# al-mcintyre/mCaller

Hardware: NVIDIA B200
Metric: per-read site calls/sec (higher is better)
Workload: dtype f64

## Files before the change

include/mcaller_b200.h:

```cpp
#ifndef MCALLER_B200_H
#define MCALLER_B200_H

#include <stdint.h>

#ifdef __cplusplus
extern "C" {
#endif

#define MC_ABI_VERSION 3

#define MC_TILE_BYTES 3840
#define MC_TEXT_PAD 4096
#define MC_MAXK 8

enum {
    MC_OK = 0,
    MC_EINVAL = -1,
    MC_ECUDA = -2,
    MC_ECAPACITY = -3
};

typedef struct mc_refindex {
    int32_t n_contigs;
    int32_t k;
// ... 96 lines not shown
    const int32_t *d_feature;
    const double *d_threshold;
    const double *d_leaf_p1;
} mc_model;

typedef struct mc_qual_entry {
    uint64_t hash;
    uint32_t check;
    uint32_t len;
    double qual;
} mc_qual_entry;


int mc_version(void);
int mc_sizeof(int what);
const char *mc_last_error(void);

int mc_read_u64(const uint64_t *d_src, int64_t n, uint64_t *h_dst, void *stream);

int mc_scan(const uint8_t *d_text, int64_t nbytes, const mc_refindex *ref, int dense,
            mc_record *d_rec, int64_t rec_cap, uint32_t *d_tile_tab , uint32_t *d_run_tab ,
            uint64_t *d_counters, void *stream);

int mc_scan_run_len(int64_t nbytes);

int mc_scan_set_run_len(int run_len);

int64_t mc_num_tiles(int64_t nbytes);

int64_t mc_workspace_bytes(int64_t n);

int mc_order_records(const uint8_t *d_text, int64_t nbytes, const mc_refindex *ref, const uint32_t *d_tile_tab, int64_t n_tiles,
                     uint32_t *d_run_tab, int run_len, const mc_record *d_rec_in, int64_t rec_in_cap, const uint64_t *d_scan_counters,
                     mc_record *d_rec_out, int64_t rec_out_cap, uint64_t *d_n_out, uint32_t *d_seg_flags ,
                     uint32_t *d_run_first , void *d_ws, void *stream);

int mc_segment_reads(const uint8_t *d_text, mc_record *d_rec, const uint64_t *d_n_records, int64_t rec_cap,
                     uint32_t *d_seg_flags , const uint32_t *d_run_first, int64_t n_runs,
                     uint32_t *d_seg_start, uint64_t *d_nseg, void *d_ws, void *stream);

int mc_segment_quality(const uint8_t *d_text, const mc_record *d_rec, const uint32_t *d_seg_start, const uint64_t *d_nseg,
                       int64_t seg_cap, const mc_qual_entry *d_table, int64_t table_size, double *d_seg_qual, uint64_t *d_err,
                       void *stream);

int mc_build_windows(const mc_record *d_rec, const uint64_t *d_n_records, int64_t rec_cap, const uint32_t *d_seg_start,
                     const uint64_t *d_nseg, int64_t seg_cap, const double *d_seg_qual, const mc_refindex *ref, int skip_thresh,
                     double qual_thresh, int two_models, mc_call *d_calls, int64_t call_cap, uint32_t *d_seg_count,
                     uint64_t *d_ncalls, void *d_ws, double *d_spill, int64_t spill_cap, void *stream);

typedef struct mc_carry {
    mc_call row;
    uint32_t valid;
    int32_t first_kept_contig;
    uint64_t chunks;
    uint64_t pad[6];
} mc_carry;
int mc_carry_reset(mc_carry *d_carry, void *stream);
int mc_carry_rows(mc_call *d_rows, const uint64_t *d_ncalls, const mc_record *d_rec, const uint64_t *d_n_records,
                  const uint32_t *d_seg_start, const uint64_t *d_nseg, const double *d_seg_qual, double qual_thresh,
                  mc_carry *d_carry, uint64_t *d_nrows_out, const uint64_t *d_abort, void *stream);
int mc_chunk_guard(const uint64_t *d_counters, int64_t rec_cap, const uint64_t *d_n_records, int64_t rec_out_cap,
                   const uint64_t *d_nseg, int64_t seg_cap, const uint64_t *d_ncalls, int64_t call_cap, uint64_t *d_abort,
                   uint64_t *d_sticky , void *stream);
int mc_carry_close(mc_carry *d_carry, int closing_contig, const int64_t *d_next_contigs, int from, int count, mc_call *d_row_out,
                   uint32_t *d_depth, uint32_t *d_meth, uint64_t *d_first, int64_t n_sites, uint64_t *d_row_base, void *stream);

int64_t mc_classify_workspace_bytes(int64_t row_cap);
int mc_classify(mc_call *d_calls, const uint64_t *d_nrows, int64_t row_cap, const mc_model *models, void *d_ws, void *stream);

int mc_hist_accumulate(const mc_call *d_calls, const uint64_t *d_nrows, int64_t row_cap, uint32_t *d_depth, uint32_t *d_meth,
                       uint64_t *d_first, int64_t n_sites, uint64_t *d_row_base, mc_call *d_odd, int64_t odd_cap, uint64_t *d_n_odd,
                       const uint64_t *d_abort , void *stream);
// ... 91 lines not shown
```

mcaller_b200/_lib.py:

```python
import ctypes as C
import os

import numpy as np

HERE = os.path.dirname(os.path.abspath(__file__))
LIB_PATH = os.environ.get("MCALLER_B200_LIB") or os.path.join(HERE, "libmcaller_b200.so")

MC_TILE_BYTES = 3840
MC_TEXT_PAD = 4096
MC_MAXK = 8
MC_C_COUNT = 16
COUNTER_NAMES = ["lines", "kept", "records", "short", "unknown_contig", "nnn", "badpos", "longline", "overflow", "run_cursor", "quiet_chunks"]

MC_ABI_VERSION = 3
MC_CALL, MC_TOO_MANY_SKIPS, MC_MULTI_M, MC_NONE = 0, 1, 2, 3
MC_CE_CONTEXT, MC_CE_MODELKEY, MC_CE_BADNUM, MC_CE_COLUMN, MC_CE_SPACING = 1, 2, 4, 8, 16
MC_MLP, MC_LR, MC_GNB, MC_RF = 0, 1, 2, 3
PENDING = 0xFFFFFFFF


class RefIndex(C.Structure):
    _fields_ = [("n_contigs", C.c_int32), ("k", C.c_int32), ("d_names", C.c_void_p), ("d_name_off", C.c_void_p),
                ("d_base", C.c_void_p), ("d_len", C.c_void_p), ("d_site_fwd", C.c_void_p), ("d_site_rev", C.c_void_p),
                ("d_cand", C.c_void_p), ("d_rank_fwd", C.c_void_p), ("d_rank_rev", C.c_void_p), ("d_bases", C.c_void_p),
# ... 36 lines not shown
                ("lr", C.c_double), ("tol", C.c_double), ("best_loss", C.c_double), ("n_iter", C.c_int32), ("no_improve", C.c_int32),
                ("stopped", C.c_int32), ("pad", C.c_int32)]


MC_TRAIN_HIDDEN, MC_TRAIN_BATCH = 100, 200

CARRY_BYTES = 192

QUAL_DTYPE = np.dtype([("hash", "<u8"), ("check", "<u4"), ("len", "<u4"), ("qual", "<f8")])
assert QUAL_DTYPE.itemsize == 24
DIFFS_ROW_DTYPE = np.dtype([("line_off", "<u8"), ("slot", "<u4"), ("values_off", "<u4"), ("values_len", "<u4"), ("prob_off", "<u4"),
                            ("prob_len", "<u4"), ("pad", "<u4")])
assert DIFFS_ROW_DTYPE.itemsize == 32


class McallerCudaError(RuntimeError):
    pass


_lib = None

_PROTOS = {
    "mc_version": (C.c_int, []),
    "mc_sizeof": (C.c_int, [C.c_int]),
    "mc_last_error": (C.c_char_p, []),
    "mc_read_u64": (C.c_int, [C.c_void_p, C.c_int64, C.c_void_p, C.c_void_p]),
    "mc_scan": (C.c_int, [C.c_void_p, C.c_int64, C.POINTER(RefIndex), C.c_int, C.c_void_p, C.c_int64, C.c_void_p, C.c_void_p, C.c_void_p,
                          C.c_void_p]),
    "mc_scan_run_len": (C.c_int, [C.c_int64]),
    "mc_scan_set_run_len": (C.c_int, [C.c_int]),
    "mc_num_tiles": (C.c_int64, [C.c_int64]),
    "mc_workspace_bytes": (C.c_int64, [C.c_int64]),
    "mc_order_records": (C.c_int, [C.c_void_p, C.c_int64, C.POINTER(RefIndex), C.c_void_p, C.c_int64, C.c_void_p, C.c_int, C.c_void_p,
                                   C.c_int64, C.c_void_p, C.c_void_p, C.c_int64, C.c_void_p, C.c_void_p, C.c_void_p, C.c_void_p, C.c_void_p]),
    "mc_segment_reads": (C.c_int, [C.c_void_p, C.c_void_p, C.c_void_p, C.c_int64, C.c_void_p, C.c_void_p, C.c_int64, C.c_void_p, C.c_void_p,
                                   C.c_void_p, C.c_void_p]),
    "mc_segment_quality": (C.c_int, [C.c_void_p, C.c_void_p, C.c_void_p, C.c_void_p, C.c_int64, C.c_void_p, C.c_int64, C.c_void_p,
                                     C.c_void_p, C.c_void_p]),
    "mc_build_windows": (C.c_int, [C.c_void_p, C.c_void_p, C.c_int64, C.c_void_p, C.c_void_p, C.c_int64, C.c_void_p, C.POINTER(RefIndex),
                                   C.c_int, C.c_double, C.c_int, C.c_void_p, C.c_int64, C.c_void_p, C.c_void_p, C.c_void_p, C.c_void_p,
                                   C.c_int64, C.c_void_p]),
    "mc_carry_reset": (C.c_int, [C.c_void_p, C.c_void_p]),
    "mc_carry_rows": (C.c_int, [C.c_void_p, C.c_void_p, C.c_void_p, C.c_void_p, C.c_void_p, C.c_void_p, C.c_void_p, C.c_double, C.c_void_p,
                                C.c_void_p, C.c_void_p, C.c_void_p]),
    "mc_chunk_guard": (C.c_int, [C.c_void_p, C.c_int64, C.c_void_p, C.c_int64, C.c_void_p, C.c_int64, C.c_void_p, C.c_int64, C.c_void_p,
                                 C.c_void_p, C.c_void_p]),
    "mc_carry_close": (C.c_int, [C.c_void_p, C.c_int, C.c_void_p, C.c_int, C.c_int, C.c_void_p, C.c_void_p, C.c_void_p, C.c_void_p,
                                 C.c_int64, C.c_void_p, C.c_void_p]),
    "mc_classify_workspace_bytes": (C.c_int64, [C.c_int64]),
    "mc_classify": (C.c_int, [C.c_void_p, C.c_void_p, C.c_int64, C.POINTER(Model), C.c_void_p, C.c_void_p]),
    "mc_hist_accumulate": (C.c_int, [C.c_void_p, C.c_void_p, C.c_int64, C.c_void_p, C.c_void_p, C.c_void_p, C.c_int64, C.c_void_p,
                                     C.c_void_p, C.c_int64, C.c_void_p, C.c_void_p, C.c_void_p]),
    "mc_count_calls": (C.c_int, [C.c_void_p, C.c_void_p, C.c_int64, C.c_void_p, C.c_void_p]),
    "mc_bed_select": (C.c_int, [C.c_void_p, C.c_void_p, C.c_int64, C.c_int64, C.c_double, C.c_int, C.c_void_p, C.c_void_p, C.c_void_p]),
    "mc_format_rows": (C.c_int64, [C.c_void_p, C.c_int64, C.c_void_p, C.c_void_p, C.c_int32, C.c_void_p, C.c_void_p, C.c_void_p, C.c_void_p,
                                   C.c_int32, C.c_int32, C.c_char_p, C.c_char_p, C.c_int32, C.c_int32, C.c_void_p, C.c_int64]),
    "mc_fastq_tiles": (C.c_int64, [C.c_int64]),
    "mc_fastq_index": (C.c_int, [C.c_void_p, C.c_int64, C.c_void_p, C.c_void_p, C.c_void_p, C.c_int64, C.c_void_p, C.c_void_p, C.c_void_p]),
    "mc_fastq_quality": (C.c_int, [C.c_void_p, C.c_int64, C.c_void_p, C.c_int64, C.c_void_p, C.c_int64, C.c_void_p, C.c_void_p, C.c_void_p,
                                   C.c_void_p]),
    "mc_synth_genome": (C.c_int, [C.POINTER(SynthSpec), C.c_void_p, C.c_int64, C.c_void_p]),
    "mc_synth_sizes": (C.c_int, [C.POINTER(SynthSpec), C.c_int64, C.c_int64, C.c_int64, C.c_void_p, C.c_void_p]),
    "mc_synth_write": (C.c_int, [C.POINTER(SynthSpec), C.c_int64, C.c_int64, C.c_int64, C.c_void_p, C.c_void_p, C.c_void_p]),
    "mc_diffs_aggregate_ex": (C.c_int, [C.c_void_p, C.c_int64, C.c_int64, C.c_void_p, C.c_int64, C.c_void_p, C.c_int64, C.c_void_p, C.c_void_p]),
    "mc_diffs_rehash": (C.c_int, [C.c_void_p, C.c_int64, C.c_void_p, C.c_int64, C.c_void_p, C.c_void_p]),
    "mc_diffs_rows": (C.c_int, [C.c_void_p, C.c_int64, C.c_void_p, C.c_int64, C.c_void_p, C.c_int64, C.c_void_p, C.c_int64, C.c_void_p,
                                C.c_void_p]),
    "mc_mlp_train_init": (C.c_int, [C.c_void_p, C.c_int32, C.c_void_p]),
    "mc_mlp_train_epochs": (C.c_int, [C.c_void_p, C.c_int32, C.c_void_p, C.c_int32, C.c_void_p]),
# ... 31 lines not shown
```

mcaller_b200/csrc/records.cu:

```cuda
#include "parse.cuh"

namespace {

constexpr int SCAN_THREADS = 256;
constexpr int SCAN_IPT = 8;
constexpr int SCAN_BLOCK = SCAN_THREADS * SCAN_IPT;

__global__ void __launch_bounds__(SCAN_THREADS) k_scan_reduce(const uint32_t *__restrict__ in, int64_t n_cap,
                                                            const unsigned long long *__restrict__ d_n,
                                                            unsigned long long *__restrict__ block_sums) {
    __shared__ int s_warp[SCAN_THREADS / 32 + 1];
    const int64_t n = d_n ? mc_dev_count(d_n, n_cap) : n_cap;
    const int64_t base = (int64_t)blockIdx.x * SCAN_BLOCK;
    unsigned long long acc = 0ull;
#pragma unroll
    for (int j = 0; j < SCAN_IPT; ++j) {
        const int64_t i = base + (int64_t)j * SCAN_THREADS + threadIdx.x;
        if (i < n) acc += in[i];
    }
    for (int d = 16; d > 0; d >>= 1) acc += __shfl_down_sync(0xffffffffu, acc, d);
    __shared__ unsigned long long s_sum[SCAN_THREADS / 32];
    if ((threadIdx.x & 31) == 0) s_sum[threadIdx.x >> 5] = acc;
    __syncthreads();
    if (threadIdx.x == 0) {
// ... 59 lines not shown
    int total;
    int off = mc_block_exscan<SCAN_THREADS>(sum, s_warp, total);
    uint32_t run = (uint32_t)block_sums[blockIdx.x] + (uint32_t)off;
#pragma unroll
    for (int j = 0; j < SCAN_IPT; ++j) {
        const int64_t i = base + j;
        if (i < n) out[i] = run;
        run += v[j];
    }
}

}

int64_t mc_exscan_ws_bytes(int64_t n) { return ((n + SCAN_BLOCK - 1) / SCAN_BLOCK + 1) * 8 + 256; }

int mc_exscan_u32(const uint32_t *d_in, uint32_t *d_out, int64_t n_cap, const uint64_t *d_n, uint64_t *d_total, void *d_ws,
                  cudaStream_t st) {
    if (n_cap <= 0) {
        if (d_total) MC_CUDA_CHECK(cudaMemsetAsync(d_total, 0, 8, st));
        return MC_OK;
    }
    const int64_t nb = (n_cap + SCAN_BLOCK - 1) / SCAN_BLOCK;
    unsigned long long *sums = reinterpret_cast<unsigned long long *>(d_ws);
    const unsigned long long *dn = reinterpret_cast<const unsigned long long *>(d_n);
    k_scan_reduce<<<(unsigned)nb, SCAN_THREADS, 0, st>>>(d_in, n_cap, dn, sums);
    MC_LAUNCH_CHECK();
    k_scan_sums<<<1, 1024, 0, st>>>(sums, nb, reinterpret_cast<unsigned long long *>(d_total));
    MC_LAUNCH_CHECK();
    k_scan_down<<<(unsigned)nb, SCAN_THREADS, 0, st>>>(d_in, n_cap, dn, sums, d_out);
    MC_LAUNCH_CHECK();
    return MC_OK;
}

extern "C" int64_t mc_windows_workspace_bytes(int64_t rec_cap);
extern "C" int64_t mc_workspace_bytes(int64_t n) {
    if (n < 1) n = 1;
    const int64_t a = ((n * 4 + 255) / 256) * 256;
    const int64_t mine = 2 * a + mc_exscan_ws_bytes(n) + 512;
    const int64_t win = mc_windows_workspace_bytes(n);
    return mine > win ? mine : win;
}
static inline uint32_t *ws_a(void *ws) { return reinterpret_cast<uint32_t *>(ws); }
static inline uint32_t *ws_b(void *ws, int64_t n) { return reinterpret_cast<uint32_t *>(reinterpret_cast<uint8_t *>(ws) + ((n * 4 + 255) / 256) * 256); }
static inline void *ws_s(void *ws, int64_t n) { return reinterpret_cast<uint8_t *>(ws) + 2 * (((n * 4 + 255) / 256) * 256); }

namespace {

__global__ void __launch_bounds__(256) k_run_resolve(uint32_t *__restrict__ run_tab, int64_t n_runs, uint32_t *__restrict__ cnt_clean,
                                                    const unsigned long long *__restrict__ scan_counters, unsigned long long rec_in_cap) {
    const int64_t r = (int64_t)blockIdx.x * blockDim.x + threadIdx.x;
    if (r >= n_runs) return;
    if (scan_counters && (scan_counters[MC_C_OVERFLOW] != 0ull || scan_counters[MC_C_RECORDS] > rec_in_cap)) {
        cnt_clean[r] = 0u;
        return;
    }
    uint32_t count = run_tab[2 * r];
    const uint32_t v = run_tab[2 * r + 1];
    if (v & 1u) {
        int64_t p = r - 1;
        uint32_t st = 0u;
        while (p >= 0 && (st = (run_tab[2 * p + 1] >> 1) & 3u) == 0u) --p;
        if (p >= 0 && st == 1u && count > 0u) {
            run_tab[2 * r + 1] = v | 0x80000000u;
            --count;
        }
    }
    cnt_clean[r] = count;
}

__global__ void __launch_bounds__(256, 4) k_gather_finish(const uint8_t *__restrict__ text, int64_t limit, mc_refindex R,
                                                      const uint32_t *__restrict__ tile_tab, const uint32_t *__restrict__ run_tab,
                                                      const uint32_t *__restrict__ run_dst, int64_t n_tiles, int64_t n_runs, int run_len,
                                                      const mc_record *__restrict__ in, unsigned long long in_cap, mc_record *__restrict__ out,
                                                      unsigned long long out_cap, uint32_t *__restrict__ seg_flags,
                                                      uint32_t *__restrict__ run_first) {
    const int lane = threadIdx.x & 31;
    const int64_t warp0 = ((int64_t)blockIdx.x * blockDim.x + threadIdx.x) >> 5, n_warps = ((int64_t)gridDim.x * blockDim.x) >> 5;
    for (int64_t run = warp0; run < n_runs; run += n_warps) {
    const uint32_t rv = __ldg(run_tab + 2 * run + 1);
    const bool empty_run = __ldg(run_dst + run) == __ldg(run_dst + run + 1);
    if (run_first && lane == 0) run_first[run] = empty_run ? 0xFFFFFFFFu : __ldg(run_dst + run);
    if (__ldg(run_tab + 2 * run) == 0u) continue;
    const bool drop = (rv >> 31) != 0u;
    unsigned long long d_run = __ldg(run_dst + run);
    const int64_t c0 = run * run_len, c1 = min(c0 + (int64_t)run_len, n_tiles);
    long long carry_line = -1;
    uint32_t carry_span = 0u;
    for (int64_t cb = c0; cb < c1; cb += 32) {
        const int64_t c = cb + lane;
        unsigned long long src = 0ull;
        uint32_t cnt = 0u;
        if (c < c1) {
            const uint2 e = __ldg(reinterpret_cast<const uint2 *>(tile_tab) + c);
            src = e.x;
            cnt = e.y & 0xFFFFu;
            if (drop && ((e.y >> 16) & 1u) && cnt > 0u) { src += 1ull; --cnt; }
        }
        uint32_t incl = cnt;
#pragma unroll
        for (int d = 1; d < 32; d <<= 1) {
            const uint32_t t = __shfl_up_sync(0xffffffffu, incl, d);
            if (lane >= d) incl += t;
        }
        const uint32_t excl = incl - cnt, tot = __shfl_sync(0xffffffffu, incl, 31);
        for (uint32_t k0 = 0; k0 < tot; k0 += 32) {
            const uint32_t idx = k0 + lane;
            const bool act = idx < tot;
            int lo = 0, hi = 31;
#pragma unroll
            for (int st = 0; st < 5; ++st) {
                const int mid = (lo + hi + 1) >> 1;
                const uint32_t e_mid = __shfl_sync(0xffffffffu, excl, mid);
                if (e_mid <= idx) lo = mid; else hi = mid - 1;
            }
            const unsigned long long s_own = __shfl_sync(0xffffffffu, src, lo);
            const uint32_t e_own = __shfl_sync(0xffffffffu, excl, lo);
            const unsigned long long slot = s_own + (idx - e_own), dst = d_run + idx;
            const bool ok = act && slot < in_cap && dst < out_cap;
            alignas(16) mc_record r;
            long long line = -1;
            uint32_t span = 0u;
            if (ok) {
                const uint4 *sp = reinterpret_cast<const uint4 *>(in + slot);
                uint4 *dr = reinterpret_cast<uint4 *>(&r);
                dr[0] = __ldg(sp);
                dr[1] = __ldg(sp + 1);
                if (r.flags & MC_RF_RAW) mc_finish_record_win(text, limit, r);
                if (r.flags & MC_RF_CAND) {
                    const int cid = r.contig;
                    if (r.pos < __ldg(R.d_len + cid)) {
                        const int64_t g = __ldg(R.d_base + cid) + r.pos;
                        r.kbits_fwd = (uint8_t)mc_kmer_bits(R.d_site_fwd, g, R.k);
                        r.kbits_rev = (uint8_t)mc_kmer_bits(R.d_site_rev, g, R.k);
                    }
                }
                line = mc_rec_line(r);
                span = (uint32_t)r.name_off | ((uint32_t)r.name_len << 16);
            }
            long long pl = __shfl_up_sync(0xffffffffu, line, 1);
            uint32_t ps = __shfl_up_sync(0xffffffffu, span, 1);
            if (lane == 0) { pl = carry_line; ps = carry_span; }
            if (ok) {
                uint32_t sf = 1u;
                if (pl >= 0) {
                    uint32_t fl = r.flags | MC_RF_SEGKNOWN;
                    sf = 0u;
                    if ((ps >> 16) != r.name_len || bytes_differ(text + pl + (ps & 0xFFFFu), text + line + r.name_off, r.name_len)) {
                        fl |= MC_RF_NEWREAD;
                        sf = 1u;
                    }
                    r.flags = (uint8_t)fl;
                }
                if (seg_flags) seg_flags[dst] = sf;
                uint4 *dp = reinterpret_cast<uint4 *>(out + dst);
                const uint4 *sr = reinterpret_cast<const uint4 *>(&r);
                dp[0] = sr[0];
                dp[1] = sr[1];
            }
            const int last = (int)min(tot - k0, 32u) - 1;
            carry_line = __shfl_sync(0xffffffffu, line, last);
            carry_span = __shfl_sync(0xffffffffu, span, last);
        }
        d_run += tot;
    }
    }
}

__global__ void __launch_bounds__(256) k_seg_flags(const uint8_t *__restrict__ text, mc_record *__restrict__ rec, int64_t n_cap,
                                                  const unsigned long long *__restrict__ d_n, uint32_t *__restrict__ flags,
                                                  const uint32_t *__restrict__ known) {
    const int64_t n = mc_dev_count(d_n, n_cap);
    const int64_t i = (int64_t)blockIdx.x * blockDim.x + threadIdx.x;
    if (i >= n) return;
    if (known) {
        const uint32_t kf = known[i];
        if (kf < 2u) { flags[i] = kf; return; }
    }
    uint32_t f = 1u;
    const mc_record b = rec[i];
    if (b.flags & MC_RF_SEGKNOWN) {
        f = (b.flags & MC_RF_NEWREAD) ? 1u : 0u;
    } else {
        if (i > 0) {
            const mc_record a = rec[i - 1];
            if (a.name_len == b.name_len)
                f = bytes_differ(text + mc_rec_line(a) + a.name_off, text + mc_rec_line(b) + b.name_off, a.name_len) ? 1u : 0u;
        }
        rec[i].flags = (uint8_t)(b.flags | MC_RF_SEGKNOWN | (f ? MC_RF_NEWREAD : 0u));
    }
    flags[i] = f;
}

__global__ void __launch_bounds__(256) k_seg_fix(const uint8_t *__restrict__ text, mc_record *__restrict__ rec, const unsigned long long *__restrict__ d_n,
                                                int64_t n_cap, const uint32_t *__restrict__ run_first, int64_t n_runs, uint32_t *__restrict__ flags) {
    const int64_t run = (int64_t)blockIdx.x * blockDim.x + threadIdx.x;
    if (run >= n_runs) return;
    const uint32_t i = run_first[run];
    if (i == 0xFFFFFFFFu || (int64_t)i >= mc_dev_count(d_n, n_cap)) return;
    uint32_t f = 1u;
    const mc_record b = rec[i];
    if (i > 0u) {
        const mc_record a = rec[i - 1];
        if (a.name_len == b.name_len)
            f = bytes_differ(text + mc_rec_line(a) + a.name_off, text + mc_rec_line(b) + b.name_off, a.name_len) ? 1u : 0u;
    }
    rec[i].flags = (uint8_t)(b.flags | MC_RF_SEGKNOWN | (f ? MC_RF_NEWREAD : 0u));
    flags[i] = f;
}

__global__ void __launch_bounds__(256) k_seg_starts(const uint32_t *__restrict__ flags, const uint32_t *__restrict__ excl, int64_t n_cap,
                                                   const unsigned long long *__restrict__ d_n, uint32_t *__restrict__ seg_start,
                                                   const unsigned long long *__restrict__ d_nseg) {
    const int64_t n = mc_dev_count(d_n, n_cap);
    const int64_t i = (int64_t)blockIdx.x * blockDim.x + threadIdx.x;
    if (i < n && flags[i]) seg_start[excl[i]] = (uint32_t)i;
    if (i == 0) seg_start[*d_nseg] = (uint32_t)n;
}

__global__ void __launch_bounds__(256) k_seg_quality(const uint8_t *__restrict__ text, const mc_record *__restrict__ rec,
                                                    const uint32_t *__restrict__ seg_start, int64_t seg_cap,
                                                    const unsigned long long *__restrict__ d_nseg,
                                                    const mc_qual_entry *__restrict__ table, unsigned long long mask,
                                                    double *__restrict__ seg_qual, unsigned long long *__restrict__ d_err) {
    const int64_t n_seg = mc_dev_count(d_nseg, seg_cap);
    const int64_t s = (int64_t)blockIdx.x * blockDim.x + threadIdx.x;
    if (s >= n_seg) return;
    const mc_record r = rec[seg_start[s]];
    const mc_read_key key = mc_read_key_of(text + mc_rec_line(r) + r.name_off, r.name_len);
    double q = __longlong_as_double(0x7ff8000000000000ll);
    unsigned long long slot = key.hash & mask;
    for (unsigned long long probe = 0; probe <= mask; ++probe) {
        const mc_qual_entry e = table[slot];
        if (e.hash == 0ull) break;
        if (e.hash == key.hash && e.check == key.check && e.len == key.len) { q = e.qual; break; }
        slot = (slot + 1) & mask;
    }
    if (q != q) atomicAdd(d_err, 1ull);
    seg_qual[s] = q;
}

}

extern "C" int mc_order_records(const uint8_t *d_text, int64_t nbytes, const mc_refindex *ref, const uint32_t *d_tile_tab, int64_t n_tiles,
                                uint32_t *d_run_tab, int run_len, const mc_record *d_rec_in, int64_t rec_in_cap,
                                const uint64_t *d_scan_counters, mc_record *d_rec_out, int64_t rec_out_cap, uint64_t *d_n_out,
                                uint32_t *d_seg_flags, uint32_t *d_run_first, void *d_ws, void *stream) {
    MC_REQUIRE(!d_seg_flags == !d_run_first, "d_seg_flags and d_run_first go together");
    MC_REQUIRE(d_text && ref && d_tile_tab && d_run_tab && d_rec_in && d_rec_out && d_n_out && d_ws, "null pointer");
    MC_REQUIRE(run_len >= 1, "run length must be >= 1");
    cudaStream_t st = (cudaStream_t)stream;
    if (n_tiles <= 0) {
        MC_CUDA_CHECK(cudaMemsetAsync(d_n_out, 0, 8, st));
        return MC_OK;
    }
    const int64_t n_runs = (n_tiles + run_len - 1) / run_len;
    uint32_t *cnt = ws_a(d_ws), *dst = ws_b(d_ws, n_runs + 1);
    MC_CUDA_CHECK(cudaMemsetAsync(cnt + n_runs, 0, 4, st));
    k_run_resolve<<<(unsigned)((n_runs + 255) / 256), 256, 0, st>>>(d_run_tab, n_runs, cnt, reinterpret_cast<const unsigned long long *>(d_scan_counters),
                                                                   (unsigned long long)rec_in_cap);
    MC_LAUNCH_CHECK();
    int rc = mc_exscan_u32(cnt, dst, n_runs + 1, nullptr, d_n_out, ws_s(d_ws, n_runs + 1), st);
    if (rc) return rc;
    int64_t gf_blocks = (n_runs * 32 + 255) / 256;
    {
        int dev = 0, sms = 0;
        MC_CUDA_CHECK(cudaGetDevice(&dev));
        MC_CUDA_CHECK(cudaDeviceGetAttribute(&sms, cudaDevAttrMultiProcessorCount, dev));
        const int64_t resident = (int64_t)sms * 4;
        if (gf_blocks > resident) gf_blocks = resident;
    }
    k_gather_finish<<<(unsigned)gf_blocks, 256, 0, st>>>(d_text, nbytes + MC_TEXT_PAD - 64, *ref, d_tile_tab, d_run_tab, dst, n_tiles,
                                                                          n_runs, run_len, d_rec_in, (unsigned long long)rec_in_cap, d_rec_out,
                                                                          (unsigned long long)rec_out_cap, d_seg_flags, d_run_first);
    MC_LAUNCH_CHECK();
    return MC_OK;
}

extern "C" int mc_segment_reads(const uint8_t *d_text, mc_record *d_rec, const uint64_t *d_n_records, int64_t rec_cap,
                                uint32_t *d_seg_flags, const uint32_t *d_run_first, int64_t n_runs, uint32_t *d_seg_start, uint64_t *d_nseg,
                                void *d_ws, void *stream) {
    MC_REQUIRE(d_text && d_rec && d_n_records && d_seg_start && d_nseg && d_ws, "null pointer");
    cudaStream_t st = (cudaStream_t)stream;
    if (rec_cap <= 0) {
        MC_CUDA_CHECK(cudaMemsetAsync(d_nseg, 0, 8, st));
        MC_CUDA_CHECK(cudaMemsetAsync(d_seg_start, 0, 4, st));
        return MC_OK;
    }
    uint32_t *flags = ws_a(d_ws), *excl = ws_b(d_ws, rec_cap);
    const unsigned nb = (unsigned)((rec_cap + 255) / 256);
    const unsigned long long *dn = reinterpret_cast<const unsigned long long *>(d_n_records);
    if (d_seg_flags && d_run_first) {
        flags = d_seg_flags;
        if (n_runs > 0) k_seg_fix<<<(unsigned)((n_runs + 255) / 256), 256, 0, st>>>(d_text, d_rec, dn, rec_cap, d_run_first, n_runs, flags);
    } else {
        k_seg_flags<<<nb, 256, 0, st>>>(d_text, d_rec, rec_cap, dn, flags, nullptr);
    }
    MC_LAUNCH_CHECK();
    int rc = mc_exscan_u32(flags, excl, rec_cap, d_n_records, d_nseg, ws_s(d_ws, rec_cap), st);
    if (rc) return rc;
    k_seg_starts<<<nb, 256, 0, st>>>(flags, excl, rec_cap, dn, d_seg_start, reinterpret_cast<const unsigned long long *>(d_nseg));
    MC_LAUNCH_CHECK();
    return MC_OK;
}

extern "C" int mc_segment_quality(const uint8_t *d_text, const mc_record *d_rec, const uint32_t *d_seg_start, const uint64_t *d_nseg,
                                  int64_t seg_cap, const mc_qual_entry *d_table, int64_t table_size, double *d_seg_qual,
                                  uint64_t *d_err, void *stream) {
    MC_REQUIRE(d_text && d_rec && d_seg_start && d_nseg && d_table && d_seg_qual && d_err, "null pointer");
    MC_REQUIRE(table_size > 0 && (table_size & (table_size - 1)) == 0, "table size must be a power of two");
    if (seg_cap <= 0) return MC_OK;
    k_seg_quality<<<(unsigned)((seg_cap + 255) / 256), 256, 0, (cudaStream_t)stream>>>(
        d_text, d_rec, d_seg_start, seg_cap, reinterpret_cast<const unsigned long long *>(d_nseg), d_table,
        (unsigned long long)(table_size - 1), d_seg_qual, reinterpret_cast<unsigned long long *>(d_err));
    MC_LAUNCH_CHECK();
    return MC_OK;
}
```

mcaller_b200/engine.py:

```python
import ctypes as C

import numpy as np
import torch

from . import _lib
from ._lib import CALL_DTYPE, CARRY_BYTES, MC_C_COUNT, MC_TEXT_PAD, RECORD_DTYPE, check

C_LINES, C_KEPT, C_RECORDS, C_SHORT, C_UNKNOWN, C_NNN, C_BADPOS, C_LONGLINE, C_OVERFLOW = range(9)

S_NSEG, S_MISSING_QUAL, S_NCALLS, S_CALL_OVERFLOW, S_ABORT, S_NREC, S_NROWS = 16, 17, 18, 19, 20, 21, 22
S_STATS = 24
S_WORDS = 32
P_ROW_BASE, P_N_ODD, P_POISON = 0, 1, 2
SPILL_CAP = 1 << 22
ODD_CAP = 1 << 16


def require_cuda():
    if not torch.cuda.is_available():
        raise _lib.McallerCudaError("mcaller_b200 needs a CUDA device (B200, sm_100a); there is no CPU fallback")


class ChunkResult(object):
    __slots__ = ("n_calls", "n_records", "n_segments", "counters", "calls_dev", "missing_quality", "stats", "nbytes")
# ... 160 lines not shown
            self.redone += 1
            attempts += 1
            if attempts > 6:
                raise _lib.McallerCudaError("chunk keeps overflowing its buffers (counters: %s)" % list(map(int, cnt[:MC_C_COUNT])))
            if cnt[C_OVERFLOW] or reserved > rec_cap:
                if rec_cap >= 2 ** 32 - 2:
                    raise _lib.McallerCudaError("chunk produces more than 2^32 records; use smaller chunks")
                rec_cap = int(min(max(reserved, rec_cap * 2 if cnt[C_OVERFLOW] and reserved <= rec_cap else 0) + slack, 2 ** 32 - 2))
                call_cap = max(call_cap, rec_cap // 8 + 1024)
            elif n_seg > seg_cap:
                seg_cap = min(n_seg + 1024, rec_cap)
            else:
                call_cap = n_calls + 1024
        if attempts:
            self.d_persist[P_POISON] = 0
        res.counters = {nm: int(cnt[i]) for i, nm in enumerate(_lib.COUNTER_NAMES)}
        res.n_records = n_rec
        res.n_segments = int(cnt[S_NSEG])
        res.missing_quality = int(cnt[S_MISSING_QUAL])
        res.n_calls = int(cnt[S_NROWS])
        res.calls_dev = self._bufs["calls"]
        v = cnt[S_STATS:S_STATS + 7]
        res.stats = dict(calls=int(v[0]), pending=int(v[1]), too_many_skips=int(v[2]), multi=int(v[3]), errors=int(v[4]), methylated=int(v[5]),
                         pending_too_many_skips=int(v[6]))
        return res

    def _launch_chunk(self, d_text, nbytes, n_tiles, rec_cap, call_cap, seg_cap, read_status=True):
        L, st = self.L, self._sptr()
        V = C.c_void_p
        tile_tab = self._buf("tile_tab", 8 * max(n_tiles, 1))
        run_len = max(int(L.mc_scan_run_len(nbytes)), 1)
        n_runs = max((n_tiles + run_len - 1) // run_len, 1)
        run_tab = self._buf("run_tab", 8 * n_runs)
        run_first = self._buf("run_first", 4 * n_runs)
        rec_a = self._buf("rec_a", 32 * rec_cap)
        rec_b = self._buf("rec_b", 32 * rec_cap)
        ws = self._buf("ws", L.mc_workspace_bytes(max(rec_cap, n_tiles)))
        seg_start = self._buf("seg_start", 4 * (rec_cap + 2))
        seg_flags = self._buf("seg_flags", 4 * rec_cap)
        seg_qual = self._buf("seg_qual", 8 * seg_cap)
        seg_count = self._buf("seg_count", 4 * seg_cap)
        calls = self._buf("calls", CALL_DTYPE.itemsize * (call_cap + 1))
        self.d_small.zero_()
        if self.scan_events is not None:
            e0, e1 = torch.cuda.Event(enable_timing=True), torch.cuda.Event(enable_timing=True)
            e0.record()
        check(L.mc_scan(V(d_text.data_ptr()), nbytes, self.ref.ref(), self.scan_mode, V(rec_a.data_ptr()), rec_cap,
                        V(tile_tab.data_ptr()), V(run_tab.data_ptr()), V(self.d_small.data_ptr()), st))
        if self.scan_events is not None:
            e1.record()
            self.scan_events.append((e0, e1))
        check(L.mc_order_records(V(d_text.data_ptr()), nbytes, self.ref.ref(), V(tile_tab.data_ptr()), n_tiles, V(run_tab.data_ptr()), run_len, V(rec_a.data_ptr()), rec_cap,
                                 V(self.d_small.data_ptr()), V(rec_b.data_ptr()), rec_cap, self._status_ptr(S_NREC), V(seg_flags.data_ptr()),
                                 V(run_first.data_ptr()), V(ws.data_ptr()), st))
        check(L.mc_segment_reads(V(d_text.data_ptr()), V(rec_b.data_ptr()), self._status_ptr(S_NREC), rec_cap, V(seg_flags.data_ptr()), V(run_first.data_ptr()),
                                 n_runs if n_tiles else 0, V(seg_start.data_ptr()),
                                 self._status_ptr(S_NSEG), V(ws.data_ptr()), st))
        check(L.mc_segment_quality(V(d_text.data_ptr()), V(rec_b.data_ptr()), V(seg_start.data_ptr()), self._status_ptr(S_NSEG), seg_cap,
                                   V(self.d_qual.data_ptr()), self.qual_table_size, V(seg_qual.data_ptr()), self._status_ptr(S_MISSING_QUAL), st))
        rows1 = V(calls.data_ptr() + CALL_DTYPE.itemsize)
        check(L.mc_build_windows(V(rec_b.data_ptr()), self._status_ptr(S_NREC), rec_cap, V(seg_start.data_ptr()), self._status_ptr(S_NSEG),
                                 seg_cap, V(seg_qual.data_ptr()), self.ref.ref(), self.skip_thresh, self.qual_thresh, self.two_models,
                                 rows1, call_cap, V(seg_count.data_ptr()), self._status_ptr(S_NCALLS), V(ws.data_ptr()),
                                 V(self.d_spill.data_ptr()), SPILL_CAP, st))
        check(L.mc_chunk_guard(V(self.d_small.data_ptr()), rec_cap, self._status_ptr(S_NREC), rec_cap, self._status_ptr(S_NSEG), seg_cap,
                               self._status_ptr(S_NCALLS), call_cap, self._status_ptr(S_ABORT), self._persist_ptr(P_POISON), st))
        check(L.mc_carry_rows(V(calls.data_ptr()), self._status_ptr(S_NCALLS), V(rec_b.data_ptr()), self._status_ptr(S_NREC),
                              V(seg_start.data_ptr()), self._status_ptr(S_NSEG), V(seg_qual.data_ptr()), self.qual_thresh,
                              V(self.d_carry.data_ptr()), self._status_ptr(S_NROWS), self._status_ptr(S_ABORT), st))
        self.launches += 1 + 5 + 5 + 1 + 7 + 2
        if self.models is not None:
            cls_ws = self._buf("cls_ws", L.mc_classify_workspace_bytes(call_cap + 1))
            check(L.mc_classify(V(calls.data_ptr()), self._status_ptr(S_NROWS), call_cap + 1, self.models.array, V(cls_ws.data_ptr()), st))
            self.launches += 2
            if self.histogram:
                check(L.mc_hist_accumulate(V(calls.data_ptr()), self._status_ptr(S_NROWS), call_cap + 1, V(self.d_depth.data_ptr()),
                                           V(self.d_meth.data_ptr()), V(self.d_first.data_ptr()), self.ref.n_sites, self._persist_ptr(P_ROW_BASE),
                                           V(self.d_odd.data_ptr()), ODD_CAP, self._persist_ptr(P_N_ODD), self._status_ptr(S_ABORT), st))
                self.launches += 2
        check(L.mc_count_calls(V(calls.data_ptr()), self._status_ptr(S_NROWS), call_cap + 1, self._status_ptr(S_STATS), st))
        self.launches += 1
        if not read_status:
            return None
        return self._read_status().copy()

    def launch_chunk(self, d_text, nbytes):
        if not self.rec_per_byte:
            raise _lib.McallerCudaError("launch_chunk needs a preceding run_chunk (capacities are learned from it)")
        n_tiles = int(self.L.mc_num_tiles(nbytes))
        rec_cap, call_cap, seg_cap = self._caps(nbytes, n_tiles)
        self._launch_chunk(d_text, nbytes, n_tiles, rec_cap, call_cap, seg_cap, read_status=False)

    def overflowed(self, clear=True):
        v = int(self.d_persist[P_POISON].item())
        if clear and v:
            self.d_persist[P_POISON] = 0
        return bool(v)

    def count_rows(self, res):
        return dict(res.stats)

    def records(self, n_rec):
        return self._bufs["rec_b"][: n_rec * 32].cpu().numpy().view(RECORD_DTYPE)
# ... 22 lines not shown
```

Baseline: 49.33 million.

## Fuse read segmentation into record ordering with a decoupled look-back scan

```diff
diff --git a/include/mcaller_b200.h b/include/mcaller_b200.h
--- a/include/mcaller_b200.h
+++ b/include/mcaller_b200.h
@@ -152,12 +152,8 @@
 
 int mc_order_records(const uint8_t *d_text, int64_t nbytes, const mc_refindex *ref, const uint32_t *d_tile_tab, int64_t n_tiles,
                      uint32_t *d_run_tab, int run_len, const mc_record *d_rec_in, int64_t rec_in_cap, const uint64_t *d_scan_counters,
-                     mc_record *d_rec_out, int64_t rec_out_cap, uint64_t *d_n_out, uint32_t *d_seg_flags ,
-                     uint32_t *d_run_first , void *d_ws, void *stream);
-
-int mc_segment_reads(const uint8_t *d_text, mc_record *d_rec, const uint64_t *d_n_records, int64_t rec_cap,
-                     uint32_t *d_seg_flags , const uint32_t *d_run_first, int64_t n_runs,
-                     uint32_t *d_seg_start, uint64_t *d_nseg, void *d_ws, void *stream);
+                     mc_record *d_rec_out, int64_t rec_out_cap, uint64_t *d_n_out, uint32_t *d_src_of ,
+                     uint32_t *d_seg_start , uint64_t *d_nseg, void *d_ws, void *stream);
 
 int mc_segment_quality(const uint8_t *d_text, const mc_record *d_rec, const uint32_t *d_seg_start, const uint64_t *d_nseg,
                        int64_t seg_cap, const mc_qual_entry *d_table, int64_t table_size, double *d_seg_qual, uint64_t *d_err,
diff --git a/mcaller_b200/_lib.py b/mcaller_b200/_lib.py
--- a/mcaller_b200/_lib.py
+++ b/mcaller_b200/_lib.py
@@ -92,9 +92,8 @@
     "mc_num_tiles": (C.c_int64, [C.c_int64]),
     "mc_workspace_bytes": (C.c_int64, [C.c_int64]),
     "mc_order_records": (C.c_int, [C.c_void_p, C.c_int64, C.POINTER(RefIndex), C.c_void_p, C.c_int64, C.c_void_p, C.c_int, C.c_void_p,
-                                   C.c_int64, C.c_void_p, C.c_void_p, C.c_int64, C.c_void_p, C.c_void_p, C.c_void_p, C.c_void_p, C.c_void_p]),
-    "mc_segment_reads": (C.c_int, [C.c_void_p, C.c_void_p, C.c_void_p, C.c_int64, C.c_void_p, C.c_void_p, C.c_int64, C.c_void_p, C.c_void_p,
-                                   C.c_void_p, C.c_void_p]),
+                                   C.c_int64, C.c_void_p, C.c_void_p, C.c_int64, C.c_void_p, C.c_void_p, C.c_void_p, C.c_void_p, C.c_void_p,
+                                   C.c_void_p]),
     "mc_segment_quality": (C.c_int, [C.c_void_p, C.c_void_p, C.c_void_p, C.c_void_p, C.c_int64, C.c_void_p, C.c_int64, C.c_void_p,
                                      C.c_void_p, C.c_void_p]),
     "mc_build_windows": (C.c_int, [C.c_void_p, C.c_void_p, C.c_int64, C.c_void_p, C.c_void_p, C.c_int64, C.c_void_p, C.POINTER(RefIndex),
diff --git a/mcaller_b200/csrc/records.cu b/mcaller_b200/csrc/records.cu
--- a/mcaller_b200/csrc/records.cu
+++ b/mcaller_b200/csrc/records.cu
@@ -115,17 +115,25 @@
     return MC_OK;
 }
 
+constexpr int FIN_BATCHES = 4;
+constexpr int FIN_TILE = 32 * FIN_BATCHES - 1;
+static inline int64_t fin_tiles(int64_t rec_cap) { return rec_cap > 0 ? (rec_cap + FIN_TILE - 1) / FIN_TILE : 1; }
+
 extern "C" int64_t mc_windows_workspace_bytes(int64_t rec_cap);
 extern "C" int64_t mc_workspace_bytes(int64_t n) {
     if (n < 1) n = 1;
     const int64_t a = ((n * 4 + 255) / 256) * 256;
-    const int64_t mine = 2 * a + mc_exscan_ws_bytes(n) + 512;
+    const int64_t mine = 2 * a + mc_exscan_ws_bytes(n) + 1024 + 8 * (fin_tiles(n) + 1);
     const int64_t win = mc_windows_workspace_bytes(n);
     return mine > win ? mine : win;
 }
 static inline uint32_t *ws_a(void *ws) { return reinterpret_cast<uint32_t *>(ws); }
 static inline uint32_t *ws_b(void *ws, int64_t n) { return reinterpret_cast<uint32_t *>(reinterpret_cast<uint8_t *>(ws) + ((n * 4 + 255) / 256) * 256); }
 static inline void *ws_s(void *ws, int64_t n) { return reinterpret_cast<uint8_t *>(ws) + 2 * (((n * 4 + 255) / 256) * 256); }
+static inline unsigned long long *fin_state(void *ws, int64_t n) {
+    const int64_t off = 2 * (((n * 4 + 255) / 256) * 256) + mc_exscan_ws_bytes(n);
+    return reinterpret_cast<unsigned long long *>(reinterpret_cast<uint8_t *>(ws) + ((off + 255) / 256) * 256);
+}
 
 namespace {
 
@@ -151,153 +159,152 @@
     cnt_clean[r] = count;
 }
 
-__global__ void __launch_bounds__(256, 4) k_gather_finish(const uint8_t *__restrict__ text, int64_t limit, mc_refindex R,
-                                                      const uint32_t *__restrict__ tile_tab, const uint32_t *__restrict__ run_tab,
-                                                      const uint32_t *__restrict__ run_dst, int64_t n_tiles, int64_t n_runs, int run_len,
-                                                      const mc_record *__restrict__ in, unsigned long long in_cap, mc_record *__restrict__ out,
-                                                      unsigned long long out_cap, uint32_t *__restrict__ seg_flags,
-                                                      uint32_t *__restrict__ run_first) {
+__global__ void __launch_bounds__(256) k_order_map(const uint32_t *__restrict__ tile_tab, const uint32_t *__restrict__ run_tab,
+                                                   const uint32_t *__restrict__ run_dst, int64_t n_tiles, int64_t n_runs, int run_len,
+                                                   uint32_t *__restrict__ src_of, unsigned long long out_cap) {
     const int lane = threadIdx.x & 31;
     const int64_t warp0 = ((int64_t)blockIdx.x * blockDim.x + threadIdx.x) >> 5, n_warps = ((int64_t)gridDim.x * blockDim.x) >> 5;
     for (int64_t run = warp0; run < n_runs; run += n_warps) {
-    const uint32_t rv = __ldg(run_tab + 2 * run + 1);
-    const bool empty_run = __ldg(run_dst + run) == __ldg(run_dst + run + 1);
-    if (run_first && lane == 0) run_first[run] = empty_run ? 0xFFFFFFFFu : __ldg(run_dst + run);
-    if (__ldg(run_tab + 2 * run) == 0u) continue;
-    const bool drop = (rv >> 31) != 0u;
-    unsigned long long d_run = __ldg(run_dst + run);
-    const int64_t c0 = run * run_len, c1 = min(c0 + (int64_t)run_len, n_tiles);
+        unsigned long long d_run = __ldg(run_dst + run);
+        if (d_run == __ldg(run_dst + run + 1)) continue;
+        const bool drop = (__ldg(run_tab + 2 * run + 1) >> 31) != 0u;
+        const int64_t c0 = run * run_len, c1 = min(c0 + (int64_t)run_len, n_tiles);
+        for (int64_t cb = c0; cb < c1; cb += 32) {
+            const int64_t c = cb + lane;
+            uint32_t src = 0u, cnt = 0u;
+            if (c < c1) {
+                const uint2 e = __ldg(reinterpret_cast<const uint2 *>(tile_tab) + c);
+                src = e.x;
+                cnt = e.y & 0xFFFFu;
+                if (drop && ((e.y >> 16) & 1u) && cnt > 0u) { src += 1u; --cnt; }
+            }
+            uint32_t incl = cnt;
+#pragma unroll
+            for (int d = 1; d < 32; d <<= 1) {
+                const uint32_t t = __shfl_up_sync(0xffffffffu, incl, d);
+                if (lane >= d) incl += t;
+            }
+            const uint32_t excl = incl - cnt, tot = __shfl_sync(0xffffffffu, incl, 31);
+            for (uint32_t k0 = 0; k0 < tot; k0 += 32) {
+                const uint32_t idx = k0 + lane;
+                int lo = 0, hi = 31;
+#pragma unroll
+                for (int st = 0; st < 5; ++st) {
+                    const int mid = (lo + hi + 1) >> 1;
+                    const uint32_t e_mid = __shfl_sync(0xffffffffu, excl, mid);
+                    if (e_mid <= idx) lo = mid; else hi = mid - 1;
+                }
+                const uint32_t s_own = __shfl_sync(0xffffffffu, src, lo);
+                const uint32_t e_own = __shfl_sync(0xffffffffu, excl, lo);
+                const unsigned long long dst = d_run + idx;
+                if (idx < tot && dst < out_cap) src_of[dst] = s_own + (idx - e_own);
+            }
+            d_run += tot;
+        }
+    }
+}
+
+constexpr unsigned long long TILE_AGG = 1ull << 32, TILE_PRE = 2ull << 32;
+
+__global__ void __launch_bounds__(256, 3) k_order_finish(const uint8_t *__restrict__ text, int64_t limit, mc_refindex R,
+                                                      const uint32_t *__restrict__ src_of, const mc_record *__restrict__ in,
+                                                      unsigned long long in_cap, mc_record *__restrict__ out, int64_t out_cap,
+                                                      const unsigned long long *__restrict__ d_n, unsigned long long *tile_state,
+                                                      unsigned long long *ticket, uint32_t *__restrict__ seg_start,
+                                                      unsigned long long *__restrict__ d_nseg) {
+    const int lane = threadIdx.x & 31;
+    const int64_t n = mc_dev_count(d_n, out_cap);
+    for (;;) {
+    unsigned long long t = 0ull;
+    if (lane == 0) t = atomicAdd(ticket, 1ull);
+    t = __shfl_sync(0xffffffffu, t, 0);
+    const int64_t i0 = (int64_t)t * FIN_TILE;
+    if (i0 >= n) {
+        if (t == 0ull && lane == 0) {
+            *d_nseg = 0ull;
+            seg_start[0] = 0u;
+        }
+        return;
+    }
+    uint32_t newread[FIN_BATCHES];
     long long carry_line = -1;
     uint32_t carry_span = 0u;
-    for (int64_t cb = c0; cb < c1; cb += 32) {
-        const int64_t c = cb + lane;
-        unsigned long long src = 0ull;
-        uint32_t cnt = 0u;
-        if (c < c1) {
-            const uint2 e = __ldg(reinterpret_cast<const uint2 *>(tile_tab) + c);
-            src = e.x;
-            cnt = e.y & 0xFFFFu;
-            if (drop && ((e.y >> 16) & 1u) && cnt > 0u) { src += 1ull; --cnt; }
-        }
-        uint32_t incl = cnt;
-#pragma unroll
-        for (int d = 1; d < 32; d <<= 1) {
-            const uint32_t t = __shfl_up_sync(0xffffffffu, incl, d);
-            if (lane >= d) incl += t;
-        }
-        const uint32_t excl = incl - cnt, tot = __shfl_sync(0xffffffffu, incl, 31);
-        for (uint32_t k0 = 0; k0 < tot; k0 += 32) {
-            const uint32_t idx = k0 + lane;
-            const bool act = idx < tot;
-            int lo = 0, hi = 31;
-#pragma unroll
-            for (int st = 0; st < 5; ++st) {
-                const int mid = (lo + hi + 1) >> 1;
-                const uint32_t e_mid = __shfl_sync(0xffffffffu, excl, mid);
-                if (e_mid <= idx) lo = mid; else hi = mid - 1;
-            }
-            const unsigned long long s_own = __shfl_sync(0xffffffffu, src, lo);
-            const uint32_t e_own = __shfl_sync(0xffffffffu, excl, lo);
-            const unsigned long long slot = s_own + (idx - e_own), dst = d_run + idx;
-            const bool ok = act && slot < in_cap && dst < out_cap;
-            alignas(16) mc_record r;
-            long long line = -1;
-            uint32_t span = 0u;
-            if (ok) {
-                const uint4 *sp = reinterpret_cast<const uint4 *>(in + slot);
-                uint4 *dr = reinterpret_cast<uint4 *>(&r);
-                dr[0] = __ldg(sp);
-                dr[1] = __ldg(sp + 1);
-                if (r.flags & MC_RF_RAW) mc_finish_record_win(text, limit, r);
-                if (r.flags & MC_RF_CAND) {
-                    const int cid = r.contig;
-                    if (r.pos < __ldg(R.d_len + cid)) {
-                        const int64_t g = __ldg(R.d_base + cid) + r.pos;
-                        r.kbits_fwd = (uint8_t)mc_kmer_bits(R.d_site_fwd, g, R.k);
-                        r.kbits_rev = (uint8_t)mc_kmer_bits(R.d_site_rev, g, R.k);
-                    }
+#pragma unroll
+    for (int b = 0; b < FIN_BATCHES; ++b) {
+        const int64_t i = i0 - 1 + 32 * b + lane;
+        const bool own = (b > 0 || lane > 0) && i < n;
+        uint32_t slot = 0xFFFFFFFFu;
+        if (i >= 0 && i < n) slot = __ldg(src_of + i);
+        const bool ok = slot < in_cap;
+        alignas(16) mc_record r;
+        long long line = -1;
+        uint32_t span = 0u;
+        if (ok) {
+            const uint4 *sp = reinterpret_cast<const uint4 *>(in + slot);
+            uint4 *dr = reinterpret_cast<uint4 *>(&r);
+            dr[0] = __ldg(sp);
+            dr[1] = __ldg(sp + 1);
+            if (r.flags & MC_RF_RAW) mc_finish_record_win(text, limit, r);
+            if (r.flags & MC_RF_CAND) {
+                const int cid = r.contig;
+                if (r.pos < __ldg(R.d_len + cid)) {
+                    const int64_t g = __ldg(R.d_base + cid) + r.pos;
+                    r.kbits_fwd = (uint8_t)mc_kmer_bits(R.d_site_fwd, g, R.k);
+                    r.kbits_rev = (uint8_t)mc_kmer_bits(R.d_site_rev, g, R.k);
                 }
-                line = mc_rec_line(r);
-                span = (uint32_t)r.name_off | ((uint32_t)r.name_len << 16);
-            }
-            long long pl = __shfl_up_sync(0xffffffffu, line, 1);
-            uint32_t ps = __shfl_up_sync(0xffffffffu, span, 1);
-            if (lane == 0) { pl = carry_line; ps = carry_span; }
-            if (ok) {
-                uint32_t sf = 1u;
-                if (pl >= 0) {
-                    uint32_t fl = r.flags | MC_RF_SEGKNOWN;
-                    sf = 0u;
-                    if ((ps >> 16) != r.name_len || bytes_differ(text + pl + (ps & 0xFFFFu), text + line + r.name_off, r.name_len)) {
-                        fl |= MC_RF_NEWREAD;
-                        sf = 1u;
-                    }
-                    r.flags = (uint8_t)fl;
-                }
-                if (seg_flags) seg_flags[dst] = sf;
-                uint4 *dp = reinterpret_cast<uint4 *>(out + dst);
-                const uint4 *sr = reinterpret_cast<const uint4 *>(&r);
-                dp[0] = sr[0];
-                dp[1] = sr[1];
-            }
-            const int last = (int)min(tot - k0, 32u) - 1;
-            carry_line = __shfl_sync(0xffffffffu, line, last);
-            carry_span = __shfl_sync(0xffffffffu, span, last);
-        }
-        d_run += tot;
-    }
-    }
-}
-
-__global__ void __launch_bounds__(256) k_seg_flags(const uint8_t *__restrict__ text, mc_record *__restrict__ rec, int64_t n_cap,
-                                                  const unsigned long long *__restrict__ d_n, uint32_t *__restrict__ flags,
-                                                  const uint32_t *__restrict__ known) {
-    const int64_t n = mc_dev_count(d_n, n_cap);
-    const int64_t i = (int64_t)blockIdx.x * blockDim.x + threadIdx.x;
-    if (i >= n) return;
-    if (known) {
-        const uint32_t kf = known[i];
-        if (kf < 2u) { flags[i] = kf; return; }
-    }
-    uint32_t f = 1u;
-    const mc_record b = rec[i];
-    if (b.flags & MC_RF_SEGKNOWN) {
-        f = (b.flags & MC_RF_NEWREAD) ? 1u : 0u;
-    } else {
-        if (i > 0) {
-            const mc_record a = rec[i - 1];
-            if (a.name_len == b.name_len)
-                f = bytes_differ(text + mc_rec_line(a) + a.name_off, text + mc_rec_line(b) + b.name_off, a.name_len) ? 1u : 0u;
-        }
-        rec[i].flags = (uint8_t)(b.flags | MC_RF_SEGKNOWN | (f ? MC_RF_NEWREAD : 0u));
-    }
-    flags[i] = f;
-}
-
-__global__ void __launch_bounds__(256) k_seg_fix(const uint8_t *__restrict__ text, mc_record *__restrict__ rec, const unsigned long long *__restrict__ d_n,
-                                                int64_t n_cap, const uint32_t *__restrict__ run_first, int64_t n_runs, uint32_t *__restrict__ flags) {
-    const int64_t run = (int64_t)blockIdx.x * blockDim.x + threadIdx.x;
-    if (run >= n_runs) return;
-    const uint32_t i = run_first[run];
-    if (i == 0xFFFFFFFFu || (int64_t)i >= mc_dev_count(d_n, n_cap)) return;
-    uint32_t f = 1u;
-    const mc_record b = rec[i];
-    if (i > 0u) {
-        const mc_record a = rec[i - 1];
-        if (a.name_len == b.name_len)
-            f = bytes_differ(text + mc_rec_line(a) + a.name_off, text + mc_rec_line(b) + b.name_off, a.name_len) ? 1u : 0u;
-    }
-    rec[i].flags = (uint8_t)(b.flags | MC_RF_SEGKNOWN | (f ? MC_RF_NEWREAD : 0u));
-    flags[i] = f;
-}
-
-__global__ void __launch_bounds__(256) k_seg_starts(const uint32_t *__restrict__ flags, const uint32_t *__restrict__ excl, int64_t n_cap,
-                                                   const unsigned long long *__restrict__ d_n, uint32_t *__restrict__ seg_start,
-                                                   const unsigned long long *__restrict__ d_nseg) {
-    const int64_t n = mc_dev_count(d_n, n_cap);
-    const int64_t i = (int64_t)blockIdx.x * blockDim.x + threadIdx.x;
-    if (i < n && flags[i]) seg_start[excl[i]] = (uint32_t)i;
-    if (i == 0) seg_start[*d_nseg] = (uint32_t)n;
+            }
+            line = mc_rec_line(r);
+            span = (uint32_t)r.name_off | ((uint32_t)r.name_len << 16);
+        }
+        long long pl = __shfl_up_sync(0xffffffffu, line, 1);
+        uint32_t ps = __shfl_up_sync(0xffffffffu, span, 1);
+        if (lane == 0) { pl = carry_line; ps = carry_span; }
+        bool nr = false;
+        if (own && ok) {
+            nr = pl < 0 || (ps >> 16) != r.name_len || bytes_differ(text + pl + (ps & 0xFFFFu), text + line + r.name_off, r.name_len);
+            r.flags = (uint8_t)(r.flags | MC_RF_SEGKNOWN | (nr ? MC_RF_NEWREAD : 0u));
+            uint4 *dp = reinterpret_cast<uint4 *>(out + i);
+            const uint4 *sr = reinterpret_cast<const uint4 *>(&r);
+            dp[0] = sr[0];
+            dp[1] = sr[1];
+        }
+        newread[b] = __ballot_sync(0xffffffffu, nr);
+        carry_line = __shfl_sync(0xffffffffu, line, 31);
+        carry_span = __shfl_sync(0xffffffffu, span, 31);
+    }
+    uint32_t count = 0u;
+#pragma unroll
+    for (int b = 0; b < FIN_BATCHES; ++b) count += __popc(newread[b]);
+
+    volatile unsigned long long *vs = tile_state;
+    uint32_t excl = 0u;
+    if (t > 0ull) {
+        if (lane == 0) vs[t] = TILE_AGG | count;
+        long long last = (long long)t - 1;
+        for (;;) {
+            const long long j = last - lane;
+            const unsigned long long v = j >= 0 ? (unsigned long long)vs[j] : TILE_PRE;
+            const unsigned pre = __ballot_sync(0xffffffffu, v >= TILE_PRE), none = __ballot_sync(0xffffffffu, v < TILE_AGG);
+            const unsigned upto = pre ? (pre & (0u - pre)) * 2u - 1u : 0xffffffffu;
+            if (none & upto) continue;
+            excl += __reduce_add_sync(0xffffffffu, ((upto >> lane) & 1u) ? (uint32_t)v : 0u);
+            if (pre) break;
+            last -= 32;
+        }
+    }
+    if (lane == 0) vs[t] = TILE_PRE | (excl + count);
+
+    uint32_t seg = excl;
+#pragma unroll
+    for (int b = 0; b < FIN_BATCHES; ++b) {
+        if ((newread[b] >> lane) & 1u) seg_start[seg + __popc(newread[b] & ((1u << lane) - 1u))] = (uint32_t)(i0 - 1 + 32 * b + lane);
+        seg += __popc(newread[b]);
+    }
+    if (lane == 0 && i0 + FIN_TILE >= n) {
+        *d_nseg = seg;
+        seg_start[seg] = (uint32_t)n;
+    }
+    }
 }
 
 __global__ void __launch_bounds__(256) k_seg_quality(const uint8_t *__restrict__ text, const mc_record *__restrict__ rec,
@@ -327,13 +334,16 @@
 extern "C" int mc_order_records(const uint8_t *d_text, int64_t nbytes, const mc_refindex *ref, const uint32_t *d_tile_tab, int64_t n_tiles,
                                 uint32_t *d_run_tab, int run_len, const mc_record *d_rec_in, int64_t rec_in_cap,
                                 const uint64_t *d_scan_counters, mc_record *d_rec_out, int64_t rec_out_cap, uint64_t *d_n_out,
-                                uint32_t *d_seg_flags, uint32_t *d_run_first, void *d_ws, void *stream) {
-    MC_REQUIRE(!d_seg_flags == !d_run_first, "d_seg_flags and d_run_first go together");
-    MC_REQUIRE(d_text && ref && d_tile_tab && d_run_tab && d_rec_in && d_rec_out && d_n_out && d_ws, "null pointer");
+                                uint32_t *d_src_of, uint32_t *d_seg_start, uint64_t *d_nseg, void *d_ws, void *stream) {
+    MC_REQUIRE(d_text && ref && d_tile_tab && d_run_tab && d_rec_in && d_rec_out && d_n_out && d_src_of && d_seg_start && d_nseg && d_ws,
+               "null pointer");
     MC_REQUIRE(run_len >= 1, "run length must be >= 1");
+    MC_REQUIRE(rec_in_cap <= 0xFFFFFFFFll && rec_out_cap <= 0xFFFFFFFEll, "record capacities must fit 32-bit indices");
     cudaStream_t st = (cudaStream_t)stream;
     if (n_tiles <= 0) {
         MC_CUDA_CHECK(cudaMemsetAsync(d_n_out, 0, 8, st));
+        MC_CUDA_CHECK(cudaMemsetAsync(d_nseg, 0, 8, st));
+        MC_CUDA_CHECK(cudaMemsetAsync(d_seg_start, 0, 4, st));
         return MC_OK;
     }
     const int64_t n_runs = (n_tiles + run_len - 1) / run_len;
@@ -344,44 +354,33 @@
     MC_LAUNCH_CHECK();
     int rc = mc_exscan_u32(cnt, dst, n_runs + 1, nullptr, d_n_out, ws_s(d_ws, n_runs + 1), st);
     if (rc) return rc;
-    int64_t gf_blocks = (n_runs * 32 + 255) / 256;
+    int64_t map_blocks = (n_runs * 32 + 255) / 256;
     {
         int dev = 0, sms = 0;
         MC_CUDA_CHECK(cudaGetDevice(&dev));
         MC_CUDA_CHECK(cudaDeviceGetAttribute(&sms, cudaDevAttrMultiProcessorCount, dev));
-        const int64_t resident = (int64_t)sms * 4;
-        if (gf_blocks > resident) gf_blocks = resident;
-    }
-    k_gather_finish<<<(unsigned)gf_blocks, 256, 0, st>>>(d_text, nbytes + MC_TEXT_PAD - 64, *ref, d_tile_tab, d_run_tab, dst, n_tiles,
-                                                                          n_runs, run_len, d_rec_in, (unsigned long long)rec_in_cap, d_rec_out,
-                                                                          (unsigned long long)rec_out_cap, d_seg_flags, d_run_first);
-    MC_LAUNCH_CHECK();
-    return MC_OK;
-}
-
-extern "C" int mc_segment_reads(const uint8_t *d_text, mc_record *d_rec, const uint64_t *d_n_records, int64_t rec_cap,
-                                uint32_t *d_seg_flags, const uint32_t *d_run_first, int64_t n_runs, uint32_t *d_seg_start, uint64_t *d_nseg,
-                                void *d_ws, void *stream) {
-    MC_REQUIRE(d_text && d_rec && d_n_records && d_seg_start && d_nseg && d_ws, "null pointer");
-    cudaStream_t st = (cudaStream_t)stream;
-    if (rec_cap <= 0) {
-        MC_CUDA_CHECK(cudaMemsetAsync(d_nseg, 0, 8, st));
-        MC_CUDA_CHECK(cudaMemsetAsync(d_seg_start, 0, 4, st));
-        return MC_OK;
-    }
-    uint32_t *flags = ws_a(d_ws), *excl = ws_b(d_ws, rec_cap);
-    const unsigned nb = (unsigned)((rec_cap + 255) / 256);
-    const unsigned long long *dn = reinterpret_cast<const unsigned long long *>(d_n_records);
-    if (d_seg_flags && d_run_first) {
-        flags = d_seg_flags;
-        if (n_runs > 0) k_seg_fix<<<(unsigned)((n_runs + 255) / 256), 256, 0, st>>>(d_text, d_rec, dn, rec_cap, d_run_first, n_runs, flags);
-    } else {
-        k_seg_flags<<<nb, 256, 0, st>>>(d_text, d_rec, rec_cap, dn, flags, nullptr);
-    }
-    MC_LAUNCH_CHECK();
-    int rc = mc_exscan_u32(flags, excl, rec_cap, d_n_records, d_nseg, ws_s(d_ws, rec_cap), st);
-    if (rc) return rc;
-    k_seg_starts<<<nb, 256, 0, st>>>(flags, excl, rec_cap, dn, d_seg_start, reinterpret_cast<const unsigned long long *>(d_nseg));
+        const int64_t resident = (int64_t)sms * 8;
+        if (map_blocks > resident) map_blocks = resident;
+    }
+    k_order_map<<<(unsigned)map_blocks, 256, 0, st>>>(d_tile_tab, d_run_tab, dst, n_tiles, n_runs, run_len, d_src_of,
+                                                      (unsigned long long)rec_out_cap);
+    MC_LAUNCH_CHECK();
+    const int64_t n_fin = fin_tiles(rec_out_cap);
+    unsigned long long *tile_state = fin_state(d_ws, n_runs + 1), *ticket = tile_state + n_fin;
+    MC_CUDA_CHECK(cudaMemsetAsync(tile_state, 0, 8 * (n_fin + 1), st));
+    int fin_blocks = 0;
+    MC_CUDA_CHECK(cudaOccupancyMaxActiveBlocksPerMultiprocessor(&fin_blocks, k_order_finish, 256, 0));
+    {
+        int dev = 0, sms = 0;
+        MC_CUDA_CHECK(cudaGetDevice(&dev));
+        MC_CUDA_CHECK(cudaDeviceGetAttribute(&sms, cudaDevAttrMultiProcessorCount, dev));
+        const int64_t resident = (int64_t)(fin_blocks > 0 ? fin_blocks : 1) * sms, needed = (n_fin + 7) / 8;
+        fin_blocks = (int)(resident < needed ? resident : needed);
+    }
+    k_order_finish<<<(unsigned)fin_blocks, 256, 0, st>>>(d_text, nbytes + MC_TEXT_PAD - 64, *ref, d_src_of, d_rec_in,
+                                                                (unsigned long long)rec_in_cap, d_rec_out, rec_out_cap,
+                                                                reinterpret_cast<const unsigned long long *>(d_n_out), tile_state, ticket,
+                                                                d_seg_start, reinterpret_cast<unsigned long long *>(d_nseg));
     MC_LAUNCH_CHECK();
     return MC_OK;
 }
diff --git a/mcaller_b200/engine.py b/mcaller_b200/engine.py
--- a/mcaller_b200/engine.py
+++ b/mcaller_b200/engine.py
@@ -216,12 +216,11 @@
         run_len = max(int(L.mc_scan_run_len(nbytes)), 1)
         n_runs = max((n_tiles + run_len - 1) // run_len, 1)
         run_tab = self._buf("run_tab", 8 * n_runs)
-        run_first = self._buf("run_first", 4 * n_runs)
         rec_a = self._buf("rec_a", 32 * rec_cap)
         rec_b = self._buf("rec_b", 32 * rec_cap)
         ws = self._buf("ws", L.mc_workspace_bytes(max(rec_cap, n_tiles)))
         seg_start = self._buf("seg_start", 4 * (rec_cap + 2))
-        seg_flags = self._buf("seg_flags", 4 * rec_cap)
+        src_of = self._buf("src_of", 4 * rec_cap)
         seg_qual = self._buf("seg_qual", 8 * seg_cap)
         seg_count = self._buf("seg_count", 4 * seg_cap)
         calls = self._buf("calls", CALL_DTYPE.itemsize * (call_cap + 1))
@@ -235,11 +234,8 @@
             e1.record()
             self.scan_events.append((e0, e1))
         check(L.mc_order_records(V(d_text.data_ptr()), nbytes, self.ref.ref(), V(tile_tab.data_ptr()), n_tiles, V(run_tab.data_ptr()), run_len, V(rec_a.data_ptr()), rec_cap,
-                                 V(self.d_small.data_ptr()), V(rec_b.data_ptr()), rec_cap, self._status_ptr(S_NREC), V(seg_flags.data_ptr()),
-                                 V(run_first.data_ptr()), V(ws.data_ptr()), st))
-        check(L.mc_segment_reads(V(d_text.data_ptr()), V(rec_b.data_ptr()), self._status_ptr(S_NREC), rec_cap, V(seg_flags.data_ptr()), V(run_first.data_ptr()),
-                                 n_runs if n_tiles else 0, V(seg_start.data_ptr()),
-                                 self._status_ptr(S_NSEG), V(ws.data_ptr()), st))
+                                 V(self.d_small.data_ptr()), V(rec_b.data_ptr()), rec_cap, self._status_ptr(S_NREC), V(src_of.data_ptr()),
+                                 V(seg_start.data_ptr()), self._status_ptr(S_NSEG), V(ws.data_ptr()), st))
         check(L.mc_segment_quality(V(d_text.data_ptr()), V(rec_b.data_ptr()), V(seg_start.data_ptr()), self._status_ptr(S_NSEG), seg_cap,
                                    V(self.d_qual.data_ptr()), self.qual_table_size, V(seg_qual.data_ptr()), self._status_ptr(S_MISSING_QUAL), st))
         rows1 = V(calls.data_ptr() + CALL_DTYPE.itemsize)
@@ -252,7 +248,7 @@
         check(L.mc_carry_rows(V(calls.data_ptr()), self._status_ptr(S_NCALLS), V(rec_b.data_ptr()), self._status_ptr(S_NREC),
                               V(seg_start.data_ptr()), self._status_ptr(S_NSEG), V(seg_qual.data_ptr()), self.qual_thresh,
                               V(self.d_carry.data_ptr()), self._status_ptr(S_NROWS), self._status_ptr(S_ABORT), st))
-        self.launches += 1 + 5 + 5 + 1 + 7 + 2
+        self.launches += 1 + 6 + 1 + 7 + 2
         if self.models is not None:
             cls_ws = self._buf("cls_ws", L.mc_classify_workspace_bytes(call_cap + 1))
             check(L.mc_classify(V(calls.data_ptr()), self._status_ptr(S_NROWS), call_cap + 1, self.models.array, V(cls_ws.data_ptr()), st))
```

Result: slower. 48.72 million, median of 6 (-1.2%).
